# Layjins/Spider

Hardware: AMD Instinct MI355X
Metric: multimodal responses/sec (text->text+image) (higher is better)
Workload: dtype bf16

## Files before the change

### include/spider_hip.h

```cpp
#ifndef SPIDER_HIP_H
#define SPIDER_HIP_H
#define SPIDER_ABI_VERSION 4

#ifdef __cplusplus
extern "C" {
#endif

int spider_abi_version(void);
const char* spider_target_arch(void);
const char* spider_last_error(void);


int spider_embed_bf16(const void* table, const int* ids, void* out, int rows, int H, int V, void* stream);

int spider_rmsnorm_bf16(const void* x, const void* res, const void* w, void* y, void* res_out, int rows, int H,
                        float eps, void* stream);

int spider_gemv_bf16(const void* W, const void* x, void* out, const void* bias, const void* res, const void* norm_w,
                     float eps, int B, int N, int K, void* stream);

int spider_gemv_swiglu_bf16(const void* W_gate_up, const void* x, void* out, const void* norm_w, float eps, int B,
                            int I, int K, void* stream);

int spider_gemv_w8(const void* Wq, const float* scale, const void* x, void* out, const void* bias, const void* res,
// ... 20 lines not shown
int spider_lm_head_argmax_bf16(const void* W, const void* x, const void* norm_w, float eps, int* out_ids, void* logits,
                               void* ws_val, void* ws_idx, int B, int V, int K, void* stream);

int spider_lm_head_argmax_proc_bf16(const void* W, const void* x, const void* norm_w, float eps, int* out_ids, void* logits,
                                    void* ws_val, void* ws_idx, const void* seen, const void* ban, const float* penalty,
                                    const int* min_new, const int* eos_ids, const int* n_eos, const int* n_hist, int B, int V,
                                    int K, void* stream);
int spider_lm_head_argmax_w8(const void* q, const void* scale, const void* x, const void* norm_w, float eps, int* out_ids,
                             void* logits, void* ws_val, void* ws_idx, int B, int V, int K, void* stream);
int spider_lm_head_argmax_proc_w8(const void* q, const void* scale, const void* x, const void* norm_w, float eps, int* out_ids,
                                  void* logits, void* ws_val, void* ws_idx, const void* seen, const void* ban,
                                  const float* penalty, const int* min_new, const int* eos_ids, const int* n_eos,
                                  const int* n_hist, int B, int V, int K, void* stream);
int spider_lm_head_argmax_w4(const void* blocks, const void* scales, const void* x, const void* norm_w, float eps, int* out_ids,
                             void* logits, void* ws_val, void* ws_idx, int B, int V, int K, void* stream);
int spider_lm_head_argmax_proc_w4(const void* blocks, const void* scales, const void* x, const void* norm_w, float eps,
                                  int* out_ids, void* logits, void* ws_val, void* ws_idx, const void* seen, const void* ban,
                                  const float* penalty, const int* min_new, const int* eos_ids, const int* n_eos,
                                  const int* n_hist, int B, int V, int K, void* stream);
int spider_decode_advance_seen_i32(const int* next_ids, int* cur_ids, int* pos, int* slot, int* kv_end, int* hist, int* n_hist,
                                   void* seen, int V, int cap, int B, void* stream);
int spider_token_bitmap_set_i32(const int* ids, void* bitmap, int B, int n, int V, void* stream);

int spider_ngram_ban_i32(const int* prompt_ids, const int* n_prompt, int pcap, const int* hist, const int* n_hist, int cap,
                         const int* ngram, const void* ban, void* ban_step, int V, int B, void* stream);
int spider_decode_advance_seen_ngram_i32(const int* next_ids, int* cur_ids, int* pos, int* slot, int* kv_end, int* hist,
                                         int* n_hist, void* seen, const int* prompt_ids, const int* n_prompt, int pcap,
                                         const int* ngram, const void* ban, void* ban_step, int V, int cap, int B, void* stream);

int spider_attn_verify_bf16(const void* q, const void* k_cache, const void* v_cache, const int* kv_beg, const int* kv_end,
                            void* out, void* ws_o, void* ws_ml, int B, int R, int n_q, int n_kv, int d, int T_max, float scale,
                            int nsplit, void* stream);
int spider_prompt_lookup_draft_i32(const int* prompt_ids, const int* n_prompt, int pcap, const int* hist, const int* n_hist,
                                   int cap, const int* ngram, const int* k_draft, int* ids, int* pos, int* slot, int* n_draft,
                                   int R, int B, void* stream);
int spider_spec_advance_draft_i32(const int* lm_out, int* ids, int* pos, int* slot, int* kv_end, int* n_draft, int* hist,
                                  int* n_hist, int cap, const int* prompt_ids, const int* n_prompt, int pcap, const int* ngram,
                                  const int* k_draft, void* counters, int R, int B, void* stream);

int spider_spec_assist_push_i32(const int* src_out, const int* src_pos, const int* src_slot, int Rs, int rs, int* t_ids, int* t_pos,
                                int* t_slot, int R, int j, int* d_ids, int* d_pos, int* d_slot, int* d_kv_end, int draft_vocab,
                                int B, void* stream);
int spider_spec_assist_advance_i32(const int* lm_out, int* ids, int* pos, int* slot, int* kv_end, const int* n_draft, int* hist,
                                   int* n_hist, int cap, void* counters, int R, int* d_ids, int* d_pos, int* d_slot, int* d_kv_end,
                                   int draft_vocab, int B, void* stream);

int spider_beam_partial_bf16(const void* logits, float* ws_ms, float* ws_val, int* ws_tok, int rows, int V, int C, int nslice,
                             void* stream);
int spider_beam_select_f32(const float* ws_ms, const float* ws_val, const int* ws_tok, float* run_scores, const int* eos_ids,
                           const int* n_eos, const int* n_hist, float* trace_score, int* trace_beam, int* trace_tok, int cap,
                           int* src_beam, int* next_ids, int B, int K, int V, int C, int nslice, void* stream);
int spider_kv_row_gather_bf16(void* k_cache, void* v_cache, void* k_tmp, void* v_tmp, const int* src_beam, const int* kv_beg,
                              const int* kv_end, int K, int R, int layers, int rows_alloc, int n_kv, int T, int d, void* stream);

int spider_sample_partial_bf16(const void* logits, const void* seen, const void* ban, const float* penalty, const int* min_new,
                               const int* eos_ids, const int* n_eos, const int* n_hist, const int* top_k, float* ws_val,
                               int* ws_tok, int rows, int V, int nslice, void* stream);
int spider_sample_select_f32(const float* ws_val, const int* ws_tok, const float* temperature, const float* top_p, const int* top_k,
                             const void* seed, const int* row0, const int* n_hist, int* next_ids, int* cand_tok, float* cand_p,
                             int* n_keep, float* u, int rows, int V, int nslice, void* stream);

int spider_logprob_rows_bf16(const void* logits, int ld, const int* targets, const void* logits_ref, int ld_ref, float* logprob,
                             float* lse, int* argmax, float* entropy, float* kl, int* argmax_ref, int rows, int V, void* stream);

int spider_rope_kv_append_bf16(const void* qkv, const int* pos, const int* slot, const float* cos_sin, void* q_out,
                               void* k_cache, void* v_cache, int B, int S, int n_q, int n_kv, int d, int T_max,
                               void* stream);
int spider_rope_kv_append_mrope_bf16(const void* qkv, const int* pos3, const int* slot, const float* cos_sin, void* q_out,
                                     void* k_cache, void* v_cache, int B, int S, int n_q, int n_kv, int d, int T_max,
                                     int sec_t, int sec_h, void* stream);

int spider_attn_decode_bf16(const void* q, const void* k_cache, const void* v_cache, const int* kv_beg,
                            const int* kv_end, void* out, void* ws_o, void* ws_ml, int B, int n_q, int n_kv, int d,
                            int T_max, float scale, int nsplit, void* stream);

int spider_attn_decode_fused_bf16(const void* qkv, const int* pos, const float* cos_sin, void* k_cache, void* v_cache,
                                  const int* kv_beg, const int* kv_end, void* out, void* ws_o, void* ws_ml,
                                  int* counters, int B, int n_q, int n_kv, int d, int T_max, float scale, int nsplit,
                                  void* stream);
int spider_set_attn_inline(int on);
int spider_set_attn_xlane(int on);
int spider_set_gemv_sched(int sched);
int spider_set_ws_inlaunch(int on);

int spider_gemv_fm_bf16(const void* Wfm, const void* x, void* out, const void* bias, const void* res, int B, int N, int K,
                        int fold_rmsnorm, float eps, void* stream);
int spider_gemv_swiglu_fm_bf16(const void* Wfm_gate_up, const void* x, void* out, int B, int I, int K, int fold_rmsnorm, float eps,
                               void* stream);
int spider_lm_head_argmax_fm_bf16(const void* Wfm, const void* x, int* out_ids, void* logits, void* ws_val, void* ws_idx, int B,
                                  int V, int K, int fold_rmsnorm, float eps, void* stream);
int spider_lm_head_argmax_fm_proc_bf16(const void* Wfm, const void* x, int* out_ids, void* logits, void* ws_val, void* ws_idx,
                                       const void* seen, const void* ban, const float* penalty, const int* min_new,
                                       const int* eos_ids, const int* n_eos, const int* n_hist, int B, int V, int K,
                                       int fold_rmsnorm, float eps, void* stream);


int spider_gemm_bf16(const void* A, const void* W, void* C, void* C32, const void* bias, const void* res,
                     const void* rowbias, int rows_per_group, int M, int N, int K, int lda, int ldc, int act,
                     float out_scale, int w_tiled, const float* res32, float* c32d, void* ws, long ws_bytes, void* stream);

int spider_gemm_ln_bf16(const void* A, const void* Wf, void* C, const float* colsum, const float* colbias, const void* res,
                        int M, int N, int K, int ldc, int act, float eps, int w_tiled, void* ws, long ws_bytes, void* stream);

int spider_xattn_fused_bf16(const void* x, const void* mq_fm, const void* mo_fm, const float* colsum, const float* colbias,
                            const void* bias_o, void* out, int B2, int n_tok, int C, int heads, int n_keys, float eps,
                            const float* x32, float* out32, void* stream);

int spider_conv2d_nhwc_bf16(const void* x, const void* w, void* y, const void* bias, const void* res,
                            const void* rowbias, int B, int Hin, int Win, int Cin, int Cout, int ks, int stride,
                            int pad, int ups, float out_scale, int w_tiled, const float* res32, float* c32d, void* ws, long ws_bytes, void* stream);

int spider_conv_nhwc_ex_bf16(const void* x, const void* w, void* y, const void* bias, const void* res,
                             const void* rowbias, int B, int Hin, int Win, int Cin, int Cout, int kh, int kw, int stride,
                             int pad_h, int pad_w, int dil, int up_h, int up_w, int act, float act_param,
                             float out_scale, int w_tiled, const float* res32, float* c32d, void* ws, long ws_bytes, void* stream);

int spider_attn_bf16(const void* q, const void* k, const void* v, void* o,
                     long q_bs, long q_hs, long q_rs, long k_bs, long k_hs, long k_rs,
                     long v_bs, long v_hs, long v_rs, long o_bs, long o_hs, long o_rs,
                     int B, int Hq, int Hkv, int Lq, int Lk, int d, float scale, int causal, int kv_off,
                     const int* kv_beg, const void* keep_bits, int blk, int q_off, void* stream);

int spider_story_key_lists_i32(const void* keep_bits, int n_keys, int N, int img0, int n_lists, int q_img0, int stride,
                               int* key_idx, int* tiles, void* stream);
int spider_attn_keylist_bf16(const void* q, const void* k, const void* v, void* o,
                             long q_bs, long q_hs, long q_rs, long k_bs, long k_hs, long k_rs,
                             long v_bs, long v_hs, long v_rs, long o_bs, long o_hs, long o_rs,
                             int B, int Hq, int Hkv, int Lq, int Lk, int d, float scale,
                             const int* key_idx, int idx_len, const int* tiles, int n_tiles, void* stream);

int spider_attn_varlen_bf16(const void* q, const void* k, const void* v, void* o, long q_rs, long k_rs, long v_rs, long o_rs,
                            int total_rows, int Hq, int Hkv, int d, float scale, const int* tiles, int n_tiles, void* stream);

int spider_rope_rows_bf16(void* x, const float* cos_sin, long row_stride, int rows, int heads, int d, void* stream);


int spider_groupnorm_nchunk(int HW);
int spider_groupnorm_nhwc_bf16(const void* x, const void* gamma, const void* beta, void* y, void* ws, int B, int HW,
                               int C, int G, float eps, int silu, void* stream);
int spider_groupnorm_cat_nhwc_bf16(const void* x1, const void* x2, const void* gamma, const void* beta, void* y, void* cat,
                                   void* ws, int B, int HW, int C1, int C2, int G, float eps, int silu, void* stream);
int spider_conv_nhwc_gn_bf16(const void* x, const void* w, void* y, const void* bias, const void* res, const void* rowbias,
                             int B, int Hin, int Win, int Cin, int Cout, int kh, int kw, int stride, int pad_h, int pad_w,
                             int dil, int up_h, int up_w, int act, float act_param, float out_scale, int w_tiled,
                             const float* res32, float* c32d, void* ws, long ws_bytes, void* stream,
                             float* gn_part, int gn_groups, int* produced);
int spider_groupnorm_stats_nhwc_bf16(const void* x, void* partial, int B, int HW, int C, int G, int nchunk, void* stream);
int spider_groupnorm_apply_nhwc_bf16(const void* x, const void* partial, int nchunk, const void* gamma, const void* beta, void* y,
                                     int B, int HW, int C, int G, float eps, int silu, void* stream);
int spider_gemm_gn_in_bf16(const void* A, const void* W, void* C, const void* bias, int M, int N, int K, int ldc, int w_tiled,
                           const float* gn_part, int nchunk, const void* gamma, const void* beta, int G, float eps, int HW,
                           float* c32d, void* stream);
int spider_layernorm_bf16(const void* x, const void* gamma, const void* beta, void* y, int rows, int C, float eps,
                          void* stream);
int spider_geglu_bf16(const void* x, void* y, int M, int inner, void* stream);
int spider_swiglu_bf16(const void* x, void* y, int M, int inner, void* stream);
int spider_concat_channels_bf16(const void* a, const void* b, void* y, long rows, int C1, int C2, void* stream);
int spider_act_bf16(const void* x, void* y, long n, int act, void* stream);
int spider_add_bf16(const void* a, const void* b, void* y, long n, void* stream);
int spider_act_ex_bf16(const void* x, void* y, long n, int act, float param, void* stream);
int spider_add_scaled_bf16(const void* a, const void* b, void* y, long n, float scale, void* stream);
int spider_axpby_bf16(const void* a, const void* b, void* y, long n, float alpha, float beta, void* stream);
int spider_mean_tokens_bf16(const void* x, void* y, int B, int T, int C, void* stream);
int spider_moe_combine_bf16(const void* const* host_xs, int E, const void* logits, int ld, void* y, int B, long per_batch,
                            void* stream);
int spider_col2im1d_f32_bf16(const float* cols, const void* bias, void* y, int B, int L_in, int k, int stride, int pad,
// ... 147 lines not shown
```

### spider_amd/csrc/attn_flash.hip

```cpp
#include "common.hpp"
#include <stdlib.h>

using namespace spider;

namespace {

struct AttnArgs {
    const h16_t* q; const h16_t* k; const h16_t* v; h16_t* o;
    long q_bs, q_hs, q_rs;
    long k_bs, k_hs, k_rs;
    long v_bs, v_hs, v_rs;
    long o_bs, o_hs, o_rs;
    int B, Hq, Hkv, Lq, Lk, d;
    float scale_log2e;
    int causal, kv_off;
    const int* kv_beg;
    const unsigned long long* keep_bits;
    int blk, q_off;
    const int* tiles;
    int n_tiles;
    const int* key_idx;
    int idx_len;
    int xcd_order;
};

__device__ __forceinline__ float partner32(float v) {
    const uint32_t u = __float_as_uint(v);
    const auto r = __builtin_amdgcn_permlane32_swap(u, u, false, false);
    return __uint_as_float((threadIdx.x & 32) ? r[0] : r[1]);
}

template <int DP>
struct Cfg {
    static constexpr int KS = DP + 8;
    static constexpr int VS = (DP == 64 || DP == 96) ? 96 : 160;
    static constexpr int NCH = (64 * DP / 8 + 255) / 256;
    static constexpr int CPR = DP / 8;
};

template <int DP, bool ONES, bool PLAIN, bool KIDX = false>
__global__ __launch_bounds__(256, (DP <= 96 ? 2 : 1)) void attn_flash_kernel(AttnArgs p) {
    using C = Cfg<DP>;
    extern __shared__ __attribute__((aligned(16))) char smem[];
    constexpr int IMG = 64 * (C::KS + C::VS);
    h16_t* const lds0 = reinterpret_cast<h16_t*>(smem);

    const int tid = threadIdx.x, lane = tid & 63, wave = tid >> 6;
    const int h32 = lane >> 5, l32 = lane & 31;
    int qt, hq, b;
    {
        const int gx = gridDim.x, gy = gridDim.y;
        const int flat = blockIdx.x + gx * (blockIdx.y + gy * blockIdx.z);
        const int L = p.xcd_order ? xcd_remap(flat, gx * gy * (int)gridDim.z) : flat;
        qt = L % gx;
        hq = (L / gx) % gy;
        b = L / (gx * gy);
    }
    const int hk = hq / (p.Hq / p.Hkv);
    int q0 = qt * 128, lq_end = p.Lq, seg_kbeg = 0, lk_end = p.Lk;
    if (!PLAIN && p.tiles) {
        const int* rec = p.tiles + 4 * qt;
        q0 = rec[0]; lq_end = rec[0] + rec[1]; seg_kbeg = rec[2]; lk_end = rec[2] + rec[3];
    }
    const int qi = q0 + wave * 32 + l32;
    const bool q_ok = qi < lq_end;

    const h16_t* qb = p.q + b * p.q_bs + hq * p.q_hs;
    const h16_t* kb = p.k + b * p.k_bs + hk * p.k_hs;
    const h16_t* vb = p.v + b * p.v_bs + hk * p.v_hs;

    h16x8 qf[DP / 16];
#pragma unroll
    for (int ks = 0; ks < DP / 16; ++ks) {
        const int dd = ks * 16 + h32 * 8;
        u32x4 t = {0u, 0u, 0u, 0u};
        if (q_ok && dd < p.d) t = *reinterpret_cast<const u32x4*>(qb + (long)qi * p.q_rs + dd);
        qf[ks] = __builtin_bit_cast(h16x8, t);
    }

    const int kbeg = PLAIN ? 0 : (p.kv_beg ? p.kv_beg[b] : seg_kbeg);
    int kend = lk_end;
    if (!PLAIN && p.causal) kend = min(kend, q0 + 128 + p.kv_off);
    const int t_begin = kbeg / 64;
    const int t_end = (kend + 63) / 64;
// ... 389 lines not shown
            for (int i = 0; i < DP / 32; ++i)
#pragma unroll
                for (int r = 0; r < 16; ++r) acc_o[i][r] *= alpha;
        }
        qk((t + 1) & 1, sn);
        float ps4[4] = {0.f, 0.f, 0.f, 0.f};
#pragma unroll
        for (int kt = 0; kt < 2; ++kt)
#pragma unroll
            for (int r = 0; r < 16; ++r) {
                const float pv = __builtin_amdgcn_exp2f(fmaf(sc[kt][r], p.scale_log2e, -m_new));
                sc[kt][r] = pv;
                if (!ONES) ps4[r & 3] += pv;
            }
        m_run = m_new;
        if (!ONES) {
            float psum = (ps4[0] + ps4[1]) + (ps4[2] + ps4[3]);
            psum += partner32(psum);
            l_run = l_run * alpha + psum;
        }
        h16x8 pf[2][2];
#pragma unroll
        for (int kt = 0; kt < 2; ++kt)
#pragma unroll
            for (int sx = 0; sx < 2; ++sx) {
                u32x4 t4;
                t4.x = pack_h16x2(sc[kt][8 * sx + 0], sc[kt][8 * sx + 1]);
                t4.y = pack_h16x2(sc[kt][8 * sx + 2], sc[kt][8 * sx + 3]);
                t4.z = pack_h16x2(sc[kt][8 * sx + 4], sc[kt][8 * sx + 5]);
                t4.w = pack_h16x2(sc[kt][8 * sx + 6], sc[kt][8 * sx + 7]);
                pf[kt][sx] = __builtin_bit_cast(h16x8, t4);
            }
        const h16_t* Vs = Vb + (t & 1) * 64 * C::VS;
#pragma unroll
        for (int db = 0; db < DP / 32; ++db) {
#pragma unroll
            for (int kt = 0; kt < 2; ++kt)
#pragma unroll
                for (int sx = 0; sx < 2; ++sx) {
                    const int r0 = kt * 32 + 16 * sx + 4 * h32 + (i16 >> 2);
                    const int c0 = db * 32 + 16 * g16 + 4 * (i16 & 3);
                    const h16_t* a0 = Vs + r0 * C::VS + c0;
                    const h16x4 lo = __builtin_amdgcn_ds_read_tr16_b64_v4i16((__attribute__((address_space(3))) h16x4*)(a0));
                    const h16x4 hi = __builtin_amdgcn_ds_read_tr16_b64_v4i16((__attribute__((address_space(3))) h16x4*)(a0 + 8 * C::VS));
                    const h16x8 vf = {lo[0], lo[1], lo[2], lo[3], hi[0], hi[1], hi[2], hi[3]};
                    acc_o[db] = mfma_32x32x16_h16(vf, pf[kt][sx], acc_o[db]);
                }
        }
        store_k(t & 1);
        store_v((t + 1) & 1);
#pragma unroll
        for (int kt = 0; kt < 2; ++kt) sc[kt] = sn[kt];
        __syncthreads();
    }

    if (ONES) {
        float l = 0.f;
#pragma unroll
        for (int db = 0; db < DP / 32; ++db)
#pragma unroll
            for (int g = 0; g < 4; ++g)
                if (db * 32 + 8 * g == p.d) l = acc_o[db][4 * g];
        l_run = __shfl(l, l32, 64);
    }
    if (q_ok) {
        const float inv = l_run > 0.f ? 1.f / l_run : 0.f;
        h16_t* ob = p.o + b * p.o_bs + hq * p.o_hs + (long)qi * p.o_rs;
#pragma unroll
        for (int db = 0; db < DP / 32; ++db)
#pragma unroll
            for (int g = 0; g < 4; ++g) {
                const int dd = db * 32 + 8 * g + 4 * h32;
                if (dd < p.d) {
                    u32x2 o2;
                    o2.x = pack_h16x2(acc_o[db][4 * g + 0] * inv, acc_o[db][4 * g + 1] * inv);
                    o2.y = pack_h16x2(acc_o[db][4 * g + 2] * inv, acc_o[db][4 * g + 3] * inv);
                    *reinterpret_cast<u32x2*>(ob + dd) = o2;
                }
            }
    }
}

#ifndef SPIDER_F16
__global__ __launch_bounds__(1024) void key_lists_kernel(const unsigned long long* __restrict__ keep, int n_keys, int N, int img0,
                                                         int q_img0, int stride, int* __restrict__ key_idx, int* __restrict__ tiles) {
    __shared__ int wsum[16];
    __shared__ int base_s;
    const int list = blockIdx.x, img = img0 + list;
    const int lane = threadIdx.x & 63, wave = threadIdx.x >> 6;
    int* out = key_idx + (size_t)list * stride;
    if (threadIdx.x == 0) base_s = 0;
    __syncthreads();
    for (int j0 = 0; j0 < n_keys; j0 += 1024) {
        const int j = j0 + threadIdx.x;
        bool vis = false;
        if (j < n_keys) vis = ((keep[j >> 6] >> (j & 63)) & 1ull) != 0ull || (j / N == img);
        const unsigned long long bal = __ballot(vis);
        const int rank = __popcll(bal & ((1ull << lane) - 1ull));
        if (lane == 0) wsum[wave] = __popcll(bal);
        __syncthreads();
        int off = base_s;
        for (int w = 0; w < wave; ++w) off += wsum[w];
        if (vis) out[off + rank] = j;
        __syncthreads();
        if (threadIdx.x == 0) {
            int tot = 0;
            for (int w = 0; w < 16; ++w) tot += wsum[w];
            base_s += tot;
        }
        __syncthreads();
    }
    const int cnt = base_s;
    const int tpl = (N + 127) / 128;
    if ((int)threadIdx.x < tpl) {
        int* rec = tiles + ((size_t)list * tpl + threadIdx.x) * 4;
        const int qs = threadIdx.x * 128;
        rec[0] = (img - q_img0) * N + qs;
        rec[1] = min(128, N - qs);
        rec[2] = list * stride;
        rec[3] = cnt;
    }
}

#endif

__global__ __launch_bounds__(256) void attn_short_kernel(AttnArgs a) {
    constexpr int VS = 72;
    __shared__ __attribute__((aligned(16))) h16_t vs_all[4][16 * VS];
    const int lane = threadIdx.x & 63, wave = threadIdx.x >> 6;
    const long total = (long)a.B * a.Hq;
    long wid = (long)blockIdx.x * 4 + wave;
    const bool live = wid < total;
    if (!live) wid = total - 1;
    const int b = (int)(wid / a.Hq), h = (int)(wid % a.Hq);
    const int r = lane & 15, g = lane >> 4;
    const h16_t* qp = a.q + (long)b * a.q_bs + (long)h * a.q_hs + (long)min(r, a.Lq - 1) * a.q_rs + 8 * g;
    const h16_t* kp = a.k + (long)b * a.k_bs + (long)h * a.k_hs + (long)min(r, a.Lk - 1) * a.k_rs + 8 * g;
    const h16_t* vp = a.v + (long)b * a.v_bs + (long)h * a.v_hs + (long)min(r, a.Lk - 1) * a.v_rs + 8 * g;
    const h16x8 q0 = *reinterpret_cast<const h16x8*>(qp), q1 = *reinterpret_cast<const h16x8*>(qp + 32);
    const h16x8 k0 = *reinterpret_cast<const h16x8*>(kp), k1 = *reinterpret_cast<const h16x8*>(kp + 32);
    const u32x4 v0 = *reinterpret_cast<const u32x4*>(vp), v1 = *reinterpret_cast<const u32x4*>(vp + 32);
    h16_t* vs = vs_all[wave];
    *reinterpret_cast<u32x4*>(vs + r * VS + 8 * g) = v0;
    *reinterpret_cast<u32x4*>(vs + r * VS + 32 + 8 * g) = v1;

    f32x4 s = {0.f, 0.f, 0.f, 0.f};
    s = mfma_16x16x32_h16(k0, q0, s);
    s = mfma_16x16x32_h16(k1, q1, s);
    float mx = -INFINITY;
#pragma unroll
    for (int i = 0; i < 4; ++i) {
        s[i] = (4 * g + i < a.Lk) ? s[i] * a.scale_log2e : -INFINITY;
        mx = fmaxf(mx, s[i]);
    }
    mx = fmaxf(mx, __shfl_xor(mx, 16, 64));
    mx = fmaxf(mx, __shfl_xor(mx, 32, 64));
    float pr[4], l = 0.f;
#pragma unroll
    for (int i = 0; i < 4; ++i) {
        const uint32_t pk = pack_h16x2(exp2f(s[i] - mx), 0.f);
        pr[i] = h16lo_to_f32(pk);
        l += pr[i];
    }
    l += __shfl_xor(l, 16, 64);
    l += __shfl_xor(l, 32, 64);
    u32x2 pp;
    pp.x = pack_h16x2(pr[0], pr[1]);
    pp.y = pack_h16x2(pr[2], pr[3]);
    const h16x4 pf = __builtin_bit_cast(h16x4, pp);

    asm volatile("s_waitcnt lgkmcnt(0)" ::: "memory");
    const float inv = 1.f / l;
    const int i16 = lane & 15;
    h16_t* op = a.o + (long)b * a.o_bs + (long)h * a.o_hs + (long)r * a.o_rs + 4 * g;
#pragma unroll
    for (int t = 0; t < 4; ++t) {
        const h16_t* va = vs + (4 * g + (i16 >> 2)) * VS + 16 * t + 4 * (i16 & 3);
        const h16x4 vf = __builtin_amdgcn_ds_read_tr16_b64_v4i16((__attribute__((address_space(3))) h16x4*)(va));
        f32x4 o = {0.f, 0.f, 0.f, 0.f};
        o = mfma_16x16x16_h16(vf, pf, o);
        if (live && r < a.Lq) {
            u32x2 w;
            w.x = pack_h16x2(o[0] * inv, o[1] * inv);
            w.y = pack_h16x2(o[2] * inv, o[3] * inv);
            *reinterpret_cast<u32x2*>(op + 16 * t) = w;
        }
    }
}

template <int DP>
int launch(const AttnArgs& a, void* stream) {
    using C = Cfg<DP>;
    dim3 grid(a.tiles ? a.n_tiles : (a.Lq + 127) / 128, a.Hq, a.B);
    const size_t smem = (size_t)2 * 64 * (C::KS + C::VS) * sizeof(h16_t);
    static const int xcd_env = [] { const char* e = getenv("SPIDER_ATTN_XCD"); return e ? atoi(e) : 1; }();
    const_cast<AttnArgs&>(a).xcd_order = xcd_env;
    if (a.key_idx) {
        if constexpr (DP == 64) {
            if (a.d < DP) attn_flash_kernel<DP, true, false, true><<<grid, 256, smem, (hipStream_t)stream>>>(a);
            else attn_flash_kernel<DP, false, false, true><<<grid, 256, smem, (hipStream_t)stream>>>(a);
            SPIDER_LAUNCH_OK();
            return 0;
        }
        spider_set_error("attn_keylist: head_dim must be <= 64");
        return -1;
    }
    const bool plain = !a.causal && !a.keep_bits && !a.kv_beg && !a.tiles;
    static const int short_env = [] { const char* e = getenv("SPIDER_ATTN_SHORT"); return e ? atoi(e) : 1; }();
    if constexpr (DP == 64) {
        if (plain && short_env && a.d == 64 && a.Lq <= 16 && a.Lk <= 16 && a.Hq == a.Hkv) {
            const long total = (long)a.B * a.Hq;
            attn_short_kernel<<<(unsigned)((total + 3) / 4), 256, 0, (hipStream_t)stream>>>(a);
            SPIDER_LAUNCH_OK();
            return 0;
        }
    }
    static const int pipe_env = [] { const char* e = getenv("SPIDER_ATTN_PIPE"); return e ? atoi(e) : 1; }();
    if (plain && pipe_env && a.Lk % 64 == 0 && a.Lk >= 128 && DP <= 96) {
        if constexpr (DP == 64) {
            if (a.d <= 48) {
                attn_flash_pipe_kernel<DP, true, 3><<<grid, 256, smem, (hipStream_t)stream>>>(a);
                SPIDER_LAUNCH_OK();
                return 0;
            }
        }
        if (a.d < DP) attn_flash_pipe_kernel<DP, true><<<grid, 256, smem, (hipStream_t)stream>>>(a);
        else attn_flash_pipe_kernel<DP, false><<<grid, 256, smem, (hipStream_t)stream>>>(a);
        SPIDER_LAUNCH_OK();
        return 0;
    }
    if (a.d < DP) {
        if (plain) attn_flash_kernel<DP, true, true><<<grid, 256, smem, (hipStream_t)stream>>>(a);
        else attn_flash_kernel<DP, true, false><<<grid, 256, smem, (hipStream_t)stream>>>(a);
    } else {
        if (plain) attn_flash_kernel<DP, false, true><<<grid, 256, smem, (hipStream_t)stream>>>(a);
        else attn_flash_kernel<DP, false, false><<<grid, 256, smem, (hipStream_t)stream>>>(a);
    }
    SPIDER_LAUNCH_OK();
    return 0;
}

}

extern "C" {

int SPIDER_FN(spider_attn)(const void* q, const void* k, const void* v, void* o,
                     long q_bs, long q_hs, long q_rs, long k_bs, long k_hs, long k_rs,
                     long v_bs, long v_hs, long v_rs, long o_bs, long o_hs, long o_rs,
                     int B, int Hq, int Hkv, int Lq, int Lk, int d, float scale, int causal, int kv_off,
                     const int* kv_beg, const void* keep_bits, int blk, int q_off, void* stream) {
    SPIDER_CHECK(B > 0 && Hq > 0 && Hkv > 0 && Hq % Hkv == 0 && Lq > 0 && Lk > 0, "attn: bad shape");
    SPIDER_CHECK(d > 0 && d % 8 == 0 && d <= 160, "attn: head_dim must be a multiple of 8 and <= 160");
    SPIDER_CHECK(q_rs % 8 == 0 && k_rs % 8 == 0 && v_rs % 8 == 0 && o_rs % 4 == 0, "attn: row strides must keep 16-byte alignment");
    SPIDER_CHECK(q_hs % 8 == 0 && k_hs % 8 == 0 && v_hs % 8 == 0 && o_hs % 4 == 0, "attn: head strides must keep 16-byte alignment");
    SPIDER_CHECK(q_bs % 8 == 0 && k_bs % 8 == 0 && v_bs % 8 == 0 && o_bs % 4 == 0, "attn: batch strides must keep 16-byte alignment");
    SPIDER_CHECK(!keep_bits || blk > 0, "attn: keep_bits needs the image block length");
    SPIDER_CHECK((long)Lk * k_rs * 2 < (1L << 32) && (long)Lk * v_rs * 2 < (1L << 32), "attn: one (batch, head) K / V view must span < 4 GiB");
    AttnArgs a{};
    a.q = (const h16_t*)q; a.k = (const h16_t*)k; a.v = (const h16_t*)v; a.o = (h16_t*)o;
    a.q_bs = q_bs; a.q_hs = q_hs; a.q_rs = q_rs; a.k_bs = k_bs; a.k_hs = k_hs; a.k_rs = k_rs;
    a.v_bs = v_bs; a.v_hs = v_hs; a.v_rs = v_rs; a.o_bs = o_bs; a.o_hs = o_hs; a.o_rs = o_rs;
    a.B = B; a.Hq = Hq; a.Hkv = Hkv; a.Lq = Lq; a.Lk = Lk; a.d = d;
    a.scale_log2e = scale * 1.4426950408889634f;
    a.causal = causal; a.kv_off = kv_off; a.kv_beg = kv_beg;
    a.keep_bits = (const unsigned long long*)keep_bits; a.blk = keep_bits ? blk : 0; a.q_off = q_off;
    if (d <= 64) return launch<64>(a, stream);
    if (d <= 96) return launch<96>(a, stream);
    if (d <= 128) return launch<128>(a, stream);
    return launch<160>(a, stream);
}

int SPIDER_FN(spider_attn_keylist)(const void* q, const void* k, const void* v, void* o,
                             long q_bs, long q_hs, long q_rs, long k_bs, long k_hs, long k_rs,
                             long v_bs, long v_hs, long v_rs, long o_bs, long o_hs, long o_rs,
                             int B, int Hq, int Hkv, int Lq, int Lk, int d, float scale,
                             const int* key_idx, int idx_len, const int* tiles, int n_tiles, void* stream) {
    SPIDER_CHECK(B > 0 && Hq > 0 && Hkv > 0 && Hq % Hkv == 0 && Lq > 0 && Lk > 0, "attn_keylist: bad shape");
    SPIDER_CHECK(d > 0 && d % 8 == 0 && d <= 64, "attn_keylist: head_dim must be a multiple of 8 and <= 64");
    SPIDER_CHECK(key_idx && tiles && idx_len > 0 && n_tiles > 0, "attn_keylist: key lists and tile records required");
    SPIDER_CHECK(q_rs % 8 == 0 && k_rs % 8 == 0 && v_rs % 8 == 0 && o_rs % 4 == 0, "attn_keylist: row strides must keep 16-byte alignment");
    SPIDER_CHECK(q_hs % 8 == 0 && k_hs % 8 == 0 && v_hs % 8 == 0 && o_hs % 4 == 0, "attn_keylist: head strides must keep 16-byte alignment");
    SPIDER_CHECK(q_bs % 8 == 0 && k_bs % 8 == 0 && v_bs % 8 == 0 && o_bs % 4 == 0, "attn_keylist: batch strides must keep 16-byte alignment");
    SPIDER_CHECK((long)Lk * k_rs * 2 < (1L << 32) && (long)Lk * v_rs * 2 < (1L << 32), "attn_keylist: one (batch, head) K / V view must span < 4 GiB");
    AttnArgs a{};
    a.q = (const h16_t*)q; a.k = (const h16_t*)k; a.v = (const h16_t*)v; a.o = (h16_t*)o;
    a.q_bs = q_bs; a.q_hs = q_hs; a.q_rs = q_rs; a.k_bs = k_bs; a.k_hs = k_hs; a.k_rs = k_rs;
    a.v_bs = v_bs; a.v_hs = v_hs; a.v_rs = v_rs; a.o_bs = o_bs; a.o_hs = o_hs; a.o_rs = o_rs;
    a.B = B; a.Hq = Hq; a.Hkv = Hkv; a.Lq = Lq; a.Lk = Lk; a.d = d;
    a.scale_log2e = scale * 1.4426950408889634f;
    a.tiles = tiles; a.n_tiles = n_tiles; a.key_idx = key_idx; a.idx_len = idx_len;
    return launch<64>(a, stream);
}

#ifndef SPIDER_F16
int spider_story_key_lists_i32(const void* keep_bits, int n_keys, int N, int img0, int n_lists, int q_img0, int stride,
                               int* key_idx, int* tiles, void* stream) {
    SPIDER_CHECK(keep_bits && key_idx && tiles && n_keys > 0 && N > 0 && n_lists > 0, "key_lists: bad arguments");
    SPIDER_CHECK(stride >= n_keys && stride % 64 == 0, "key_lists: stride must cover the keys and be a multiple of 64");
    SPIDER_CHECK((N + 127) / 128 <= 1024, "key_lists: image block too long");
    key_lists_kernel<<<n_lists, 1024, 0, (hipStream_t)stream>>>((const unsigned long long*)keep_bits, n_keys, N, img0, q_img0, stride,
                                                               key_idx, tiles);
    SPIDER_LAUNCH_OK();
    return 0;
}

#endif

int SPIDER_FN(spider_attn_varlen)(const void* q, const void* k, const void* v, void* o, long q_rs, long k_rs, long v_rs, long o_rs,
                            int total_rows, int Hq, int Hkv, int d, float scale, const int* tiles, int n_tiles, void* stream) {
    SPIDER_CHECK(total_rows > 0 && Hq > 0 && Hkv > 0 && Hq % Hkv == 0 && n_tiles > 0 && tiles, "attn_varlen: bad shape");
    SPIDER_CHECK(d > 0 && d % 8 == 0 && d <= 160, "attn_varlen: head_dim must be a multiple of 8 and <= 160");
    SPIDER_CHECK(q_rs % 8 == 0 && k_rs % 8 == 0 && v_rs % 8 == 0 && o_rs % 4 == 0, "attn_varlen: row strides must keep 16-byte alignment");
    SPIDER_CHECK((long)total_rows * k_rs * 2 < (1L << 32) && (long)total_rows * v_rs * 2 < (1L << 32), "attn_varlen: K / V views must span < 4 GiB");
    AttnArgs a{};
    a.q = (const h16_t*)q; a.k = (const h16_t*)k; a.v = (const h16_t*)v; a.o = (h16_t*)o;
    a.q_hs = a.k_hs = a.v_hs = a.o_hs = d;
    a.q_rs = q_rs; a.k_rs = k_rs; a.v_rs = v_rs; a.o_rs = o_rs;
    a.B = 1; a.Hq = Hq; a.Hkv = Hkv; a.Lq = total_rows; a.Lk = total_rows; a.d = d;
    a.scale_log2e = scale * 1.4426950408889634f;
    a.tiles = tiles; a.n_tiles = n_tiles;
    if (d <= 64) return launch<64>(a, stream);
    if (d <= 96) return launch<96>(a, stream);
    if (d <= 128) return launch<128>(a, stream);
    return launch<160>(a, stream);
}

}
```

### spider_amd/lib.py

```python
from __future__ import annotations

import ctypes as C
import os
import threading

import torch

_HERE = os.path.dirname(os.path.abspath(__file__))
LIB_PATH = os.path.join(_HERE, "libspider_hip.so")

_lib = None
_lock = threading.Lock()

_vp, _i, _f, _l = C.c_void_p, C.c_int, C.c_float, C.c_long

SIGNATURES = {
    "spider_abi_version": (_i, []),
    "spider_target_arch": (C.c_char_p, []),
    "spider_last_error": (C.c_char_p, []),
    "spider_embed_bf16": (_i, [_vp, _vp, _vp, _i, _i, _i, _vp]),
    "spider_rmsnorm_bf16": (_i, [_vp, _vp, _vp, _vp, _vp, _i, _i, _f, _vp]),
    "spider_gemv_bf16": (_i, [_vp, _vp, _vp, _vp, _vp, _vp, _f, _i, _i, _i, _vp]),
    "spider_gemv_swiglu_bf16": (_i, [_vp, _vp, _vp, _vp, _f, _i, _i, _i, _vp]),
    "spider_gemv_w8": (_i, [_vp, _vp, _vp, _vp, _vp, _vp, _vp, _f, _i, _i, _i, _vp]),
    "spider_gemv_swiglu_w8": (_i, [_vp, _vp, _vp, _vp, _vp, _f, _i, _i, _i, _vp]),
    "spider_gemv_w4": (_i, [_vp, _vp, _vp, _vp, _vp, _vp, _vp, _f, _i, _i, _i, _vp]),
    "spider_gemv_swiglu_w4": (_i, [_vp, _vp, _vp, _vp, _vp, _f, _i, _i, _i, _vp]),
    "spider_gemv_fm_w4": (_i, [_vp, _vp, _vp, _vp, _vp, _vp, _i, _i, _i, _vp]),
    "spider_gemv_swiglu_fm_w4": (_i, [_vp, _vp, _vp, _vp, _i, _i, _i, _vp]),
    "spider_gemv_fm_w8": (_i, [_vp, _vp, _vp, _vp, _vp, _vp, _i, _i, _i, _vp]),
    "spider_gemv_swiglu_fm_w8": (_i, [_vp, _vp, _vp, _vp, _i, _i, _i, _vp]),
    "spider_lm_head_nparts": (_i, [_i]),
    "spider_decode_advance_i32": (_i, [_vp] * 7 + [_i, _i, _vp]),
    "spider_lm_head_argmax_bf16": (_i, [_vp, _vp, _vp, _f, _vp, _vp, _vp, _vp, _i, _i, _i, _vp]),
    "spider_lm_head_argmax_proc_bf16": (_i, [_vp, _vp, _vp, _f] + [_vp] * 11 + [_i, _i, _i, _vp]),
    "spider_lm_head_argmax_w8": (_i, [_vp, _vp, _vp, _vp, _f, _vp, _vp, _vp, _vp, _i, _i, _i, _vp]),
    "spider_lm_head_argmax_proc_w8": (_i, [_vp, _vp, _vp, _vp, _f] + [_vp] * 11 + [_i, _i, _i, _vp]),
    "spider_lm_head_argmax_w4": (_i, [_vp, _vp, _vp, _vp, _f, _vp, _vp, _vp, _vp, _i, _i, _i, _vp]),
    "spider_lm_head_argmax_proc_w4": (_i, [_vp, _vp, _vp, _vp, _f] + [_vp] * 11 + [_i, _i, _i, _vp]),
    "spider_decode_advance_seen_i32": (_i, [_vp] * 8 + [_i, _i, _i, _vp]),
    "spider_token_bitmap_set_i32": (_i, [_vp, _vp, _i, _i, _i, _vp]),
    "spider_ngram_ban_i32": (_i, [_vp, _vp, _i, _vp, _vp, _i, _vp, _vp, _vp, _i, _i, _vp]),
    "spider_decode_advance_seen_ngram_i32": (_i, [_vp] * 10 + [_i] + [_vp] * 3 + [_i] * 3 + [_vp]),
    "spider_beam_partial_bf16": (_i, [_vp] * 4 + [_i] * 4 + [_vp]),
    "spider_beam_select_f32": (_i, [_vp] * 10 + [_i, _vp, _vp] + [_i] * 5 + [_vp]),
    "spider_kv_row_gather_bf16": (_i, [_vp] * 7 + [_i] * 7 + [_vp]),
    "spider_sample_partial_bf16": (_i, [_vp] * 11 + [_i] * 3 + [_vp]),
    "spider_sample_select_f32": (_i, [_vp] * 13 + [_i] * 3 + [_vp]),
    "spider_logprob_rows_bf16": (_i, [_vp, _i, _vp, _vp, _i] + [_vp] * 6 + [_i, _i, _vp]),
    "spider_gemv_fm_bf16": (_i, [_vp, _vp, _vp, _vp, _vp, _i, _i, _i, _i, _f, _vp]),
    "spider_gemv_swiglu_fm_bf16": (_i, [_vp, _vp, _vp, _i, _i, _i, _i, _f, _vp]),
    "spider_lm_head_argmax_fm_bf16": (_i, [_vp, _vp, _vp, _vp, _vp, _vp, _i, _i, _i, _i, _f, _vp]),
    "spider_lm_head_argmax_fm_proc_bf16": (_i, [_vp] * 13 + [_i, _i, _i, _i, _f, _vp]),
    "spider_rope_kv_append_bf16": (_i, [_vp, _vp, _vp, _vp, _vp, _vp, _vp, _i, _i, _i, _i, _i, _i, _vp]),
    "spider_rope_kv_append_mrope_bf16": (_i, [_vp, _vp, _vp, _vp, _vp, _vp, _vp, _i, _i, _i, _i, _i, _i, _i, _i, _vp]),
    "spider_attn_decode_bf16": (_i, [_vp, _vp, _vp, _vp, _vp, _vp, _vp, _vp, _i, _i, _i, _i, _i, _f, _i, _vp]),
    "spider_attn_decode_fused_bf16": (_i, [_vp] * 11 + [_i, _i, _i, _i, _i, _f, _i, _vp]),
    "spider_attn_verify_bf16": (_i, [_vp] * 8 + [_i] * 6 + [_f, _i, _vp]),
    "spider_prompt_lookup_draft_i32": (_i, [_vp, _vp, _i, _vp, _vp, _i] + [_vp] * 6 + [_i, _i, _vp]),
    "spider_spec_advance_draft_i32": (_i, [_vp] * 8 + [_i, _vp, _vp, _i, _vp, _vp, _vp, _i, _i, _vp]),
    "spider_spec_assist_push_i32": (_i, [_vp, _vp, _vp, _i, _i, _vp, _vp, _vp, _i, _i, _vp, _vp, _vp, _vp, _i, _i, _vp]),
    "spider_spec_assist_advance_i32": (_i, [_vp] * 8 + [_i, _vp, _i] + [_vp] * 4 + [_i, _i, _vp]),
    "spider_set_attn_inline": (_i, [_i]),
    "spider_set_attn_xlane": (_i, [_i]),
    "spider_set_gemv_sched": (_i, [_i]),
    "spider_set_ws_inlaunch": (_i, [_i]),
    "spider_gemm_bf16": (_i, [_vp, _vp, _vp, _vp, _vp, _vp, _vp, _i, _i, _i, _i, _i, _i, _i, _f, _i, _vp, _vp, _vp, _l, _vp]),
    "spider_gemm_ln_bf16": (_i, [_vp, _vp, _vp, _vp, _vp, _vp, _i, _i, _i, _i, _i, _f, _i, _vp, _l, _vp]),
    "spider_xattn_fused_bf16": (_i, [_vp, _vp, _vp, _vp, _vp, _vp, _vp, _i, _i, _i, _i, _i, _f, _vp, _vp, _vp]),
    "spider_conv2d_nhwc_bf16": (_i, [_vp, _vp, _vp, _vp, _vp, _vp, _i, _i, _i, _i, _i, _i, _i, _i, _i, _f, _i, _vp, _vp, _vp, _l, _vp]),
    "spider_conv_nhwc_ex_bf16": (_i, [_vp] * 6 + [_i] * 14 + [_f, _f, _i, _vp, _vp, _vp, _l, _vp]),
    "spider_attn_bf16": (_i, [_vp, _vp, _vp, _vp] + [_l] * 12 + [_i] * 6 + [_f, _i, _i, _vp, _vp, _i, _i, _vp]),
    "spider_story_key_lists_i32": (_i, [_vp, _i, _i, _i, _i, _i, _i, _vp, _vp, _vp]),
    "spider_attn_keylist_bf16": (_i, [_vp, _vp, _vp, _vp] + [_l] * 12 + [_i] * 6 + [_f, _vp, _i, _vp, _i, _vp]),
    "spider_attn_varlen_bf16": (_i, [_vp, _vp, _vp, _vp, _l, _l, _l, _l, _i, _i, _i, _i, _f, _vp, _i, _vp]),
    "spider_rope_rows_bf16": (_i, [_vp, _vp, _l, _i, _i, _i, _vp]),
    "spider_groupnorm_nchunk": (_i, [_i]),
    "spider_groupnorm_nhwc_bf16": (_i, [_vp, _vp, _vp, _vp, _vp, _i, _i, _i, _i, _f, _i, _vp]),
    "spider_groupnorm_cat_nhwc_bf16": (_i, [_vp] * 7 + [_i, _i, _i, _i, _i, _f, _i, _vp]),
    "spider_conv_nhwc_gn_bf16": (_i, [_vp] * 6 + [_i] * 14 + [_f, _f, _i, _vp, _vp, _vp, _l, _vp] + [_vp, _i, _vp]),
    "spider_groupnorm_stats_nhwc_bf16": (_i, [_vp, _vp, _i, _i, _i, _i, _i, _vp]),
    "spider_groupnorm_apply_nhwc_bf16": (_i, [_vp, _vp, _i, _vp, _vp, _vp, _i, _i, _i, _i, _f, _i, _vp]),
    "spider_gemm_gn_in_bf16": (_i, [_vp, _vp, _vp, _vp, _i, _i, _i, _i, _i, _vp, _i, _vp, _vp, _i, _f, _i, _vp, _vp]),
    "spider_layernorm_bf16": (_i, [_vp, _vp, _vp, _vp, _i, _i, _f, _vp]),
    "spider_geglu_bf16": (_i, [_vp, _vp, _i, _i, _vp]),
    "spider_swiglu_bf16": (_i, [_vp, _vp, _i, _i, _vp]),
    "spider_concat_channels_bf16": (_i, [_vp, _vp, _vp, _l, _i, _i, _vp]),
    "spider_act_bf16": (_i, [_vp, _vp, _l, _i, _vp]),
    "spider_add_bf16": (_i, [_vp, _vp, _vp, _l, _vp]),
    "spider_act_ex_bf16": (_i, [_vp, _vp, _l, _i, _f, _vp]),
    "spider_add_scaled_bf16": (_i, [_vp, _vp, _vp, _l, _f, _vp]),
    "spider_axpby_bf16": (_i, [_vp, _vp, _vp, _l, _f, _f, _vp]),
    "spider_mean_tokens_bf16": (_i, [_vp, _vp, _i, _i, _i, _vp]),
    "spider_moe_combine_bf16": (_i, [_vp, _i, _vp, _i, _vp, _i, _l, _vp]),
    "spider_col2im1d_f32_bf16": (_i, [_vp, _vp, _vp, _i, _i, _i, _i, _i, _i, _vp]),
    "spider_l2_normalize_rows_bf16": (_i, [_vp, _vp, _i, _i, _f, _vp]),
    "spider_conv2d_small_cin_bf16": (_i, [_vp, _vp, _vp, _vp, _i, _i, _i, _i, _i, _i, _vp]),
    "spider_conv2d_small_cout_bf16": (_i, [_vp, _vp, _vp, _vp, _vp, _i, _i, _i, _i, _i, _i, _vp]),
    "spider_latent_to_nhwc_bf16": (_i, [_vp, _vp, _i, _i, _i, _i, _f, _vp]),
    "spider_cfg_combine_f32": (_i, [_vp, _vp, _i, _i, _i, _f, _vp]),
    "spider_lincomb_f32": (_i, [_vp, _vp, _i, _vp, _l, _vp]),
    "spider_softmax_rows_f32_bf16": (_i, [_vp, _vp, _i, _i, _i, _f, _vp]),
    "spider_pack_keep_bits_f32": (_i, [_vp, _vp, _i, _i, _f, _vp]),
    "spider_nhwc_to_nchw_f32": (_i, [_vp, _vp, _i, _i, _i, _f, _f, _i, _vp]),
    "spider_gemm_a32_bf16": (_i, [_vp] * 5 + [_i] * 5 + [_f, _i, _vp, _vp, _vp, _l, _vp]),
    "spider_gemm_ln_a32_bf16": (_i, [_vp] * 6 + [_i, _i, _i, _i, _i, _f, _i, _vp]),
    "spider_gemm_gn_in_a32_bf16": (_i, [_vp, _vp, _vp, _vp, _i, _i, _i, _i, _i, _vp, _i, _vp, _vp, _i, _f, _i, _vp, _vp]),
    "spider_conv_nhwc_a32_bf16": (_i, [_vp] * 6 + [_i] * 13 + [_f, _i, _vp, _vp, _vp, _l, _vp]),
    "spider_groupnorm_f32in_nhwc_bf16": (_i, [_vp, _vp, _i, _vp, _vp, _vp, _vp, _vp, _i, _i, _i, _i, _f, _i, _vp]),
    "spider_split_hilo_f32_bf16": (_i, [_vp, _vp, _vp, _l, _vp]),
    "spider_row_split_f32_bf16": (_i, [_vp, _vp, _vp, _vp, _l, _i, _f, _vp]),
    "spider_groupnorm_f32in_split_nhwc_bf16": (_i, [_vp, _vp, _i, _vp, _vp, _vp, _vp, _i, _i, _i, _i, _f, _i, _vp]),
    "spider_conv2d_small_cin_f32in_bf16": (_i, [_vp] * 5 + [_i] * 6 + [_vp]),
    "spider_conv2d_small_cout_f32in_bf16": (_i, [_vp] * 4 + [_i] * 6 + [_vp]),
    "spider_latent_to_nhwc_f32": (_i, [_vp, _vp, _i, _i, _i, _i, _f, _vp]),
    "spider_clip_preprocess": (_i, [_vp] * 5 + [_i, _vp, _vp, _i, _vp] + [_i] * 7 + [_vp]),
    "spider_safety_decide": (_i, [_vp] * 7 + [_i] * 5 + [_vp]),
    "spider_image_blackout_f32": (_i, [_vp, _vp, _i, _l, _vp]),
    "spider_logmel_tile_frames": (_i, []),
    "spider_logmel_f32": (_i, [_vp] * 8 + [_i] * 8 + [_vp]),
    "spider_qwen_image_patches": (_i, [_vp] * 6 + [_i] * 4 + [_l] + [_i] * 2 + [_vp]),
}

F16_OPS = (
    "spider_gemm", "spider_gemm_ln", "spider_xattn_fused", "spider_conv2d_nhwc", "spider_conv_nhwc_ex", "spider_attn",
    "spider_conv_nhwc_gn", "spider_groupnorm_stats_nhwc", "spider_groupnorm_apply_nhwc", "spider_gemm_gn_in",
    "spider_attn_keylist", "spider_attn_varlen", "spider_groupnorm_nhwc", "spider_groupnorm_cat_nhwc", "spider_layernorm",
    "spider_geglu", "spider_swiglu", "spider_concat_channels", "spider_act", "spider_add", "spider_act_ex", "spider_add_scaled",
    "spider_axpby", "spider_mean_tokens", "spider_moe_combine", "spider_col2im1d_f32", "spider_l2_normalize_rows",
    "spider_conv2d_small_cin", "spider_conv2d_small_cout", "spider_latent_to_nhwc", "spider_softmax_rows_f32",
    "spider_gemm_a32", "spider_gemm_ln_a32", "spider_gemm_gn_in_a32", "spider_conv_nhwc_a32", "spider_groupnorm_f32in_nhwc", "spider_conv2d_small_cin_f32in",
    "spider_conv2d_small_cout_f32in", "spider_split_hilo_f32", "spider_row_split_f32", "spider_groupnorm_f32in_split_nhwc",
)
for _n in F16_OPS:
    SIGNATURES[_n + "_f16"] = SIGNATURES[_n + "_bf16"]


class SpiderHipError(RuntimeError):
    pass


def load():
    global _lib
    if _lib is not None:
        return _lib
    with _lock:
        if _lib is not None:
# ... 24 lines not shown
```

Before: 2.044.

## Add key-split causal flash attention kernel with two key groups per block

Adds a causal prefill attention kernel for head dim 128 that runs 512 threads per block as two 256-thread key groups. The groups process alternating key tiles with register-staged double-buffered loads, then merge their softmax states through shared memory. The aim is more parallelism and latency hiding per query tile in causal attention, at the cost of doubled LDS, one block per CU and an extra merge step. It is enabled by default via an env/setter toggle, only for unmasked self-causal calls.

Result: no change. 2.052, median of 3 (+0.4%).

```diff
diff --git a/include/spider_hip.h b/include/spider_hip.h
--- a/include/spider_hip.h
+++ b/include/spider_hip.h
@@ -126,6 +126,7 @@
 int spider_set_attn_xlane(int on);
 int spider_set_gemv_sched(int sched);
 int spider_set_ws_inlaunch(int on);
+int spider_set_attn_causal_pipe(int on);
 
 int spider_gemv_fm_bf16(const void* Wfm, const void* x, void* out, const void* bias, const void* res, int B, int N, int K,
                         int fold_rmsnorm, float eps, void* stream);
diff --git a/spider_amd/csrc/attn_flash.hip b/spider_amd/csrc/attn_flash.hip
--- a/spider_amd/csrc/attn_flash.hip
+++ b/spider_amd/csrc/attn_flash.hip
@@ -1,5 +1,6 @@
 #include "common.hpp"
 #include <stdlib.h>
+#include <type_traits>
 
 using namespace spider;
 
@@ -555,6 +556,252 @@
 }
 
 #ifndef SPIDER_F16
+template <int DP>
+__global__ __launch_bounds__(512, 1) void attn_causal_split_kernel(AttnArgs p) {
+    using C = Cfg<DP>;
+    constexpr int GRP = 2;
+    constexpr int NT = 256, QR = 128;
+    constexpr int NCH = 64 * C::CPR / NT;
+    constexpr int RPI = NT / C::CPR;
+    constexpr int IMG = 2 * 64 * (C::KS + C::VS);
+    static_assert(64 * C::CPR % NT == 0 && NT % C::CPR == 0, "a key group stages whole chunk rounds");
+    extern __shared__ __attribute__((aligned(16))) char smem[];
+    const int lane = threadIdx.x & 63;
+    const int kg = __builtin_amdgcn_readfirstlane(threadIdx.x >> 8);
+    const int tid = threadIdx.x & 255, wave = __builtin_amdgcn_readfirstlane(tid >> 6);
+    h16_t* const Kb = reinterpret_cast<h16_t*>(smem) + kg * IMG;
+    h16_t* const Vb = Kb + 2 * 64 * C::KS;
+    const int h32 = lane >> 5, l32 = lane & 31;
+
+    const int nq = gridDim.x, G = p.Hq / p.Hkv, NG = p.B * p.Hkv, S = G * nq;
+    int kvg, j;
+    {
+        const int flat = blockIdx.x + nq * (blockIdx.y + (int)gridDim.y * blockIdx.z);
+        const int xcd = flat & 7, idx = flat >> 3;
+        if (p.xcd_order && NG <= 8 && 8 % NG == 0 && S % (8 / NG) == 0) {
+            const int X = 8 / NG;
+            kvg = xcd / X;
+            j = idx * X + xcd % X;
+        } else if (p.xcd_order && NG % 8 == 0) {
+            const int Y = NG / 8;
+            kvg = xcd * Y + idx % Y;
+            j = idx / Y;
+        } else {
+            kvg = flat % NG;
+            j = flat / NG;
+        }
+    }
+    const int qt = nq - 1 - j / G;
+    const int b = kvg / p.Hkv, hk = kvg % p.Hkv, hq = hk * G + j % G;
+    const int q0 = qt * QR;
+    const int wave_q0 = q0 + wave * 32;
+    const int qi = wave_q0 + l32;
+    const bool q_ok = qi < p.Lq;
+    const h16_t* qb = p.q + b * p.q_bs + hq * p.q_hs;
+    const h16_t* kb = p.k + b * p.k_bs + hk * p.k_hs;
+    const h16_t* vb = p.v + b * p.v_bs + hk * p.v_hs;
+
+    h16x8 qf[DP / 16];
+#pragma unroll
+    for (int ks = 0; ks < DP / 16; ++ks) {
+        u32x4 t = {0u, 0u, 0u, 0u};
+        if (q_ok) t = *reinterpret_cast<const u32x4*>(qb + (long)qi * p.q_rs + ks * 16 + h32 * 8);
+        qf[ks] = __builtin_bit_cast(h16x8, t);
+    }
+    const int lk_end = p.Lk;
+    const int nt = (min(lk_end, q0 + QR + p.kv_off) + 63) / 64;
+    const int wnt = min(nt, (wave_q0 + 31 + p.kv_off) / 64 + 1);
+    const int caus_max = qi + p.kv_off;
+
+    f32x16 acc_o[DP / 32];
+#pragma unroll
+    for (int i = 0; i < DP / 32; ++i)
+#pragma unroll
+        for (int r = 0; r < 16; ++r) acc_o[i][r] = 0.f;
+    float m_run = -1e30f, l_run = 0.f;
+
+    auto span = [&](long rs) { const long b_ = ((long)(lk_end - 1) * rs + p.d) * 2; return (uint32_t)(b_ < 0xFFFFFFFFl ? b_ : 0xFFFFFFFFl); };
+    const __amdgpu_buffer_rsrc_t rsrc_k = __builtin_amdgcn_make_buffer_rsrc(const_cast<h16_t*>(kb), 0, span(p.k_rs), 0x00020000);
+    const __amdgpu_buffer_rsrc_t rsrc_v = __builtin_amdgcn_make_buffer_rsrc(const_cast<h16_t*>(vb), 0, span(p.v_rs), 0x00020000);
+    u32x4 rk[NCH], rv[NCH];
+    const int ld_row = tid / C::CPR, ld_ch = tid % C::CPR;
+    auto load_k = [&](int t) {
+        const uint32_t tinv = (uint32_t)((nt - 1 - t) >> 31);
+#pragma unroll
+        for (int i = 0; i < NCH; ++i)
+            rk[i] = __builtin_bit_cast(u32x4, __builtin_amdgcn_raw_buffer_load_b128(rsrc_k, ((uint32_t)(t * 64 + ld_row + i * RPI) * (uint32_t)p.k_rs * 2u + (uint32_t)ld_ch * 16u) | tinv, 0, 0));
+    };
+    auto load_v = [&](int t) {
+        const uint32_t tinv = (uint32_t)((nt - 1 - t) >> 31);
+#pragma unroll
+        for (int i = 0; i < NCH; ++i)
+            rv[i] = __builtin_bit_cast(u32x4, __builtin_amdgcn_raw_buffer_load_b128(rsrc_v, ((uint32_t)(t * 64 + ld_row + i * RPI) * (uint32_t)p.v_rs * 2u + (uint32_t)ld_ch * 16u) | tinv, 0, 0));
+    };
+    auto store_k = [&](int buf) {
+        h16_t* Kd = Kb + buf * 64 * C::KS + ld_row * C::KS + ld_ch * 8;
+#pragma unroll
+        for (int i = 0; i < NCH; ++i) *reinterpret_cast<u32x4*>(Kd + i * RPI * C::KS) = rk[i];
+    };
+    auto store_v = [&](int buf) {
+        h16_t* Vd = Vb + buf * 64 * C::VS + ld_row * C::VS + ld_ch * 8;
+#pragma unroll
+        for (int i = 0; i < NCH; ++i) *reinterpret_cast<u32x4*>(Vd + i * RPI * C::VS) = rv[i];
+    };
+    auto qk = [&](int buf, f32x16 (&s)[2]) {
+        const h16_t* Ks = Kb + buf * 64 * C::KS;
+#pragma unroll
+        for (int kt = 0; kt < 2; ++kt) {
+#pragma unroll
+            for (int r = 0; r < 16; ++r) s[kt][r] = 0.f;
+            const h16_t* krow = Ks + (kt * 32 + l32) * C::KS + h32 * 8;
+#pragma unroll
+            for (int ks = 0; ks < DP / 16; ++ks) {
+                const h16x8 kf = *reinterpret_cast<const h16x8*>(krow + ks * 16);
+                s[kt] = mfma_32x32x16_h16(kf, qf[ks], s[kt]);
+            }
+        }
+    };
+
+    auto T = [&](int s_) { return GRP * s_ + kg; };
+    const int nsteps = (nt + GRP - 1) / GRP;
+    load_k(T(0)); load_v(T(0));
+    store_k(0); store_v(0);
+#pragma unroll
+    for (int ks = 0; ks < DP / 16; ++ks) asm volatile("" ::"v"(qf[ks]));
+    __syncthreads();
+
+    const int g16 = (lane >> 4) & 1, i16 = lane & 15;
+    auto tile = [&](int t, int st, auto masked_tag) {
+        constexpr bool MASKED = decltype(masked_tag)::value;
+        float tmax, m_sub;
+        f32x16 sc[2];
+        qk(st & 1, sc);
+        if (!MASKED) {
+            float tm[4] = {sc[0][0], sc[0][1], sc[0][2], sc[0][3]};
+#pragma unroll
+            for (int kt = 0; kt < 2; ++kt)
+#pragma unroll
+                for (int r = 0; r < 16; ++r) tm[r & 3] = fmaxf(tm[r & 3], sc[kt][r]);
+            tmax = fmaxf(fmaxf(tm[0], tm[1]), fmaxf(tm[2], tm[3]));
+            tmax = fmaxf(tmax, partner32(tmax)) * p.scale_log2e;
+        } else {
+            const int key0 = t * 64 + 4 * h32;
+            const int hi_lim = min(lk_end, caus_max + 1);
+            float tm[4] = {-1e30f, -1e30f, -1e30f, -1e30f};
+#pragma unroll
+            for (int kt = 0; kt < 2; ++kt)
+#pragma unroll
+                for (int r = 0; r < 16; ++r) {
+                    const int key = key0 + kt * 32 + (r & 3) + 8 * (r >> 2);
+                    const float sv = key < hi_lim ? sc[kt][r] * p.scale_log2e : -1e30f;
+                    sc[kt][r] = sv;
+                    tm[r & 3] = fmaxf(tm[r & 3], sv);
+                }
+            tmax = fmaxf(fmaxf(tm[0], tm[1]), fmaxf(tm[2], tm[3]));
+            tmax = fmaxf(tmax, partner32(tmax));
+        }
+        const float m_new = fmaxf(m_run, tmax);
+        const float alpha = __builtin_amdgcn_exp2f(m_run - m_new);
+        m_sub = (MASKED && m_new < -1e29f) ? 0.f : m_new;
+        if (__any(alpha != 1.f)) {
+#pragma unroll
+            for (int i = 0; i < DP / 32; ++i)
+#pragma unroll
+                for (int r = 0; r < 16; ++r) acc_o[i][r] *= alpha;
+        }
+        float ps4[4] = {0.f, 0.f, 0.f, 0.f};
+#pragma unroll
+        for (int kt = 0; kt < 2; ++kt)
+#pragma unroll
+            for (int r = 0; r < 16; ++r) {
+                const float pv = MASKED ? __builtin_amdgcn_exp2f(sc[kt][r] - m_sub)
+                                        : __builtin_amdgcn_exp2f(fmaf(sc[kt][r], p.scale_log2e, -m_sub));
+                sc[kt][r] = pv;
+                ps4[r & 3] += pv;
+            }
+        m_run = m_new;
+        float psum = (ps4[0] + ps4[1]) + (ps4[2] + ps4[3]);
+        psum += partner32(psum);
+        l_run = l_run * alpha + psum;
+        h16x8 pf[2][2];
+#pragma unroll
+        for (int kt = 0; kt < 2; ++kt)
+#pragma unroll
+            for (int sx = 0; sx < 2; ++sx) {
+                u32x4 t4;
+                t4.x = pack_h16x2(sc[kt][8 * sx + 0], sc[kt][8 * sx + 1]);
+                t4.y = pack_h16x2(sc[kt][8 * sx + 2], sc[kt][8 * sx + 3]);
+                t4.z = pack_h16x2(sc[kt][8 * sx + 4], sc[kt][8 * sx + 5]);
+                t4.w = pack_h16x2(sc[kt][8 * sx + 6], sc[kt][8 * sx + 7]);
+                pf[kt][sx] = __builtin_bit_cast(h16x8, t4);
+            }
+        const h16_t* Vs = Vb + (st & 1) * 64 * C::VS;
+#pragma unroll
+        for (int db = 0; db < DP / 32; ++db) {
+#pragma unroll
+            for (int kt = 0; kt < 2; ++kt)
+#pragma unroll
+                for (int sx = 0; sx < 2; ++sx) {
+                    const int r0 = kt * 32 + 16 * sx + 4 * h32 + (i16 >> 2);
+                    const int c0 = db * 32 + 16 * g16 + 4 * (i16 & 3);
+                    const h16_t* a0 = Vs + r0 * C::VS + c0;
+                    const h16x4 lo = __builtin_amdgcn_ds_read_tr16_b64_v4i16((__attribute__((address_space(3))) h16x4*)(a0));
+                    const h16x4 hi = __builtin_amdgcn_ds_read_tr16_b64_v4i16((__attribute__((address_space(3))) h16x4*)(a0 + 8 * C::VS));
+                    const h16x8 vf = {lo[0], lo[1], lo[2], lo[3], hi[0], hi[1], hi[2], hi[3]};
+                    acc_o[db] = mfma_32x32x16_h16(vf, pf[kt][sx], acc_o[db]);
+                }
+        }
+    };
+
+    for (int st = 0; st < nsteps; ++st) {
+        const int t = T(st);
+        load_k(T(st + 1));
+        load_v(T(st + 1));
+        if (t < wnt) {
+            if (t * 64 + 63 <= wave_q0 + p.kv_off && t * 64 + 64 <= lk_end) tile(t, st, std::false_type{});
+            else tile(t, st, std::true_type{});
+        }
+        store_k((st + 1) & 1);
+        store_v((st + 1) & 1);
+        __syncthreads();
+    }
+
+    {
+        float* const xch = reinterpret_cast<float*>(smem);
+        if (kg == 1) {
+            xch[0 * 256 + tid] = m_run;
+            xch[1 * 256 + tid] = l_run;
+#pragma unroll
+            for (int i = 0; i < DP / 32; ++i)
+#pragma unroll
+                for (int r = 0; r < 16; ++r) xch[(2 + i * 16 + r) * 256 + tid] = acc_o[i][r];
+        }
+        __syncthreads();
+        if (kg != 0) return;
+        const float m1 = xch[0 * 256 + tid], l1 = xch[1 * 256 + tid];
+        const float m = fmaxf(m_run, m1);
+        const float a0 = __builtin_amdgcn_exp2f(m_run - m), a1 = __builtin_amdgcn_exp2f(m1 - m);
+        l_run = l_run * a0 + l1 * a1;
+#pragma unroll
+        for (int i = 0; i < DP / 32; ++i)
+#pragma unroll
+            for (int r = 0; r < 16; ++r) acc_o[i][r] = acc_o[i][r] * a0 + xch[(2 + i * 16 + r) * 256 + tid] * a1;
+    }
+    if (q_ok) {
+        const float inv = l_run > 0.f ? 1.f / l_run : 0.f;
+        h16_t* ob = p.o + b * p.o_bs + hq * p.o_hs + (long)qi * p.o_rs;
+#pragma unroll
+        for (int db = 0; db < DP / 32; ++db)
+#pragma unroll
+            for (int g = 0; g < 4; ++g) {
+                u32x2 o2;
+                o2.x = pack_h16x2(acc_o[db][4 * g + 0] * inv, acc_o[db][4 * g + 1] * inv);
+                o2.y = pack_h16x2(acc_o[db][4 * g + 2] * inv, acc_o[db][4 * g + 3] * inv);
+                *reinterpret_cast<u32x2*>(ob + db * 32 + 8 * g + 4 * h32) = o2;
+            }
+    }
+}
+
 __global__ __launch_bounds__(1024) void key_lists_kernel(const unsigned long long* __restrict__ keep, int n_keys, int N, int img0,
                                                          int q_img0, int stride, int* __restrict__ key_idx, int* __restrict__ tiles) {
     __shared__ int wsum[16];
@@ -661,6 +908,14 @@
     }
 }
 
+#ifndef SPIDER_F16
+int g_attn_causal_pipe = -1;
+int attn_causal_pipe() {
+    if (g_attn_causal_pipe < 0) { const char* e = getenv("SPIDER_ATTN_CAUSAL_PIPE"); g_attn_causal_pipe = e ? (atoi(e) != 0) : 1; }
+    return g_attn_causal_pipe;
+}
+#endif
+
 template <int DP>
 int launch(const AttnArgs& a, void* stream) {
     using C = Cfg<DP>;
@@ -702,6 +957,17 @@
         SPIDER_LAUNCH_OK();
         return 0;
     }
+#ifndef SPIDER_F16
+    if constexpr (DP == 128) {
+        if (attn_causal_pipe() && a.causal && !a.keep_bits && !a.kv_beg && !a.tiles && a.d == DP && a.kv_off >= 0 && a.kv_off == a.Lk - a.Lq) {
+            static unsigned done = 0;
+            raise_dynamic_lds(&attn_causal_split_kernel<DP>, (int)(2 * smem), done);
+            attn_causal_split_kernel<DP><<<grid, 512, 2 * smem, (hipStream_t)stream>>>(a);
+            SPIDER_LAUNCH_OK();
+            return 0;
+        }
+    }
+#endif
     if (a.d < DP) {
         if (plain) attn_flash_kernel<DP, true, true><<<grid, 256, smem, (hipStream_t)stream>>>(a);
         else attn_flash_kernel<DP, true, false><<<grid, 256, smem, (hipStream_t)stream>>>(a);
@@ -766,6 +1032,12 @@
 }
 
 #ifndef SPIDER_F16
+int spider_set_attn_causal_pipe(int on) {
+    const int prev = attn_causal_pipe();
+    g_attn_causal_pipe = on != 0;
+    return prev;
+}
+
 int spider_story_key_lists_i32(const void* keep_bits, int n_keys, int N, int img0, int n_lists, int q_img0, int stride,
                                int* key_idx, int* tiles, void* stream) {
     SPIDER_CHECK(keep_bits && key_idx && tiles && n_keys > 0 && N > 0 && n_lists > 0, "key_lists: bad arguments");
diff --git a/spider_amd/lib.py b/spider_amd/lib.py
--- a/spider_amd/lib.py
+++ b/spider_amd/lib.py
@@ -63,6 +63,7 @@
     "spider_spec_assist_advance_i32": (_i, [_vp] * 8 + [_i, _vp, _i] + [_vp] * 4 + [_i, _i, _vp]),
     "spider_set_attn_inline": (_i, [_i]),
     "spider_set_attn_xlane": (_i, [_i]),
+    "spider_set_attn_causal_pipe": (_i, [_i]),
     "spider_set_gemv_sched": (_i, [_i]),
     "spider_set_ws_inlaunch": (_i, [_i]),
     "spider_gemm_bf16": (_i, [_vp, _vp, _vp, _vp, _vp, _vp, _vp, _i, _i, _i, _i, _i, _i, _i, _f, _i, _vp, _vp, _vp, _l, _vp]),
```
